# auduno/headtrackr

Hardware: NVIDIA H100
Metric: frames/sec @640x480 (detect+CAMShift) (higher is better)
Workload: dtype u8+f64

## Files before the change

headtrackr_b200/csrc/ht_api.cu:

```cuda
#include "../../include/headtrackr_b200.h"

#include <cuda.h>
#include <cuda_runtime.h>

#include <algorithm>
#include <cassert>
#include <cmath>
#include <cstdarg>
#include <cstddef>
#include <cstdio>
#include <cstdlib>
#include <cstring>
#include <map>
#include <memory>
#include <string>
#include <tuple>
#include <utility>
#include <vector>

#include "ht_common.cuh"
#include "ht_detect.cuh"
#include "ht_track.cuh"

using namespace ht;
// ... 507 lines not shown
  DevBuf d_tracker_state, d_tracker_params, d_tracker_events, d_tracker_wb;
  bool tracker_on = false;
  DevBuf d_debug, d_debug_tab;
  std::vector<DebugCanvas> h_debug;
  int debug_count = 0;
  int stroke_flags = 0, stroke_count = 0;
  DevBuf d_camera;
  std::vector<CameraCtl> h_camera;
  int camera_count = 0;
  DevBuf d_crop;
  std::vector<FaceCrop> h_crop;
  int crop_count = 0, crop_tiles = 0;
  DevBuf d_feed_table, d_feed_draw, d_feed_canvas;
  DevBuf d_ingest_recs;
  PinnedHost h_feed_table;
  Event feed_copied;
  DevBuf d_track_cost;
  DevBuf d_records, d_record_status;
  int track_heavy_div = 128;
  int track_heavy_cluster = 8;
  int track_mid_div = 32, track_mid_cluster = 4;
  Stream tier_stream[3];
  Event tier_done[3];
  int track_mask_frames = 4;
  int track_mask_min = 4;
  Event sched_ready;
  DevBuf d_sched;

  int fail(int code, const char *fmt, ...) {
    char buf[512];
    va_list ap; va_start(ap, fmt); vsnprintf(buf, sizeof(buf), fmt, ap); va_end(ap);
    err = buf;
    return code;
  }
};

#define CK(call)                                                                                   \
  do {                                                                                             \
    cudaError_t e_ = (call);                                                                       \
    if (e_ != cudaSuccess) return ctx->fail(HT_ERR_CUDA, "%s: %s", #call, cudaGetErrorString(e_)); \
  } while (0)

namespace {

bool is_device_ptr(const void *p) {
  if (!p) return false;
  cudaPointerAttributes a{};
  if (cudaPointerGetAttributes(&a, p) != cudaSuccess) { cudaGetLastError(); return false; }
// ... 96 lines not shown
  const bool on_device = is_device_ptr(slots);
  if (!on_device) {
    std::vector<uint8_t> seen((size_t)ctx->cfg.max_frames, 0);
    for (int i = 0; i < n; ++i) {
      if (slots[i] < 0 || slots[i] >= ctx->cfg.max_frames) return ctx->fail(HT_ERR_ARG, "slot %d out of range", slots[i]);
      if (seen[(size_t)slots[i]]++) return ctx->fail(HT_ERR_ARG, "slot %d appears twice in one batch", slots[i]);
    }
    CK(ctx->d_slots.reserve(sizeof(int32_t) * ctx->cfg.max_frames));
  }
  return stage_input(ctx, st, slots, on_device, sizeof(int32_t) * n, ctx->d_slots, d_slots);
}

int ensure_tracker_buffers(ht_ctx *ctx, cudaStream_t st) {
  const size_t mf = (size_t)ctx->cfg.max_frames;
  if (!ctx->model_hist.p) {
    CK(ctx->model_hist.reserve(mf * 4096 * sizeof(uint32_t)));
    CK(ctx->cur_hist.reserve(2 * mf * 4096 * sizeof(uint32_t)));
    CK(ctx->track_state.reserve(mf * sizeof(TrackState)));
    CK(cudaMemsetAsync(ctx->track_state.p, 0, mf * sizeof(TrackState), st));
    CK(ctx->d_rects.reserve(mf * 4 * sizeof(int32_t)));
    CK(ctx->d_found.reserve(mf * sizeof(int32_t)));
    CK(ctx->d_objs.reserve(mf * 6 * sizeof(int32_t)));
    CK(ctx->d_windows.reserve(mf * 4 * sizeof(int32_t)));
    CK(ctx->d_sched.reserve(2 * mf * sizeof(int32_t)));
    CK(ctx->d_track_cost.reserve(2 * mf * sizeof(int32_t)));
    CK(cudaMemsetAsync(ctx->d_track_cost.p, 0, 2 * mf * sizeof(int32_t), st));
    if (ctx->track_trace) {
      CK(ctx->d_trace.reserve(12 * mf * sizeof(unsigned long long)));
      CK(cudaMemsetAsync(ctx->d_trace.p, 0, 12 * mf * sizeof(unsigned long long), st));
    }
  }
  return HT_OK;
}

int launch_hist(ht_ctx *ctx, cudaStream_t st, const uint8_t *d_rgba, int n, int w, int h, uint32_t *hist, uint16_t *bins,
                const uint8_t *enable = nullptr) {
  const int n_px = w * h;
  int chunks = 1;
  if (n < 4 * ctx->sms) chunks = std::min(64, std::max(1, 8 * ctx->sms / n));
  if (chunks > 1) CK(cudaMemsetAsync(hist, 0, (size_t)n * 4096 * sizeof(uint32_t), st));
  ctx->prof_begin(HT_PROF_HIST, st);
  k_hist<<<dim3(chunks, n), 256, 0, st>>>(d_rgba, (size_t)n_px * 4, n_px, hist, bins, chunks, enable);
  ctx->prof_end(st);
  ++ctx->launches;
  CK(cudaGetLastError());
  return HT_OK;
}

using TrackKernel = void (*)(const uint16_t *, int, int, const int32_t *, const uint32_t *, const uint32_t *, TrackState *,
                             int, int32_t *, int32_t *, int32_t *, unsigned long long *, const int32_t *, int,
                             unsigned long long *, size_t, int, int, int32_t *, const uint8_t *);

template <int NT>
TrackKernel track_kernel(int c) {
  switch (c) {
    case 1: return k_track<1, NT>;
    case 2: return k_track<2, NT>;
    case 4: return k_track<4, NT>;
    case 16: return k_track<16, NT>;
    default: return k_track<8, NT>;
  }
}
TrackKernel track_kernel(int c, int nt) {
  return nt == 512 ? track_kernel<512>(c) : nt == 128 ? track_kernel<128>(c) : track_kernel<256>(c);
}

struct TrackArgs {
  const uint16_t *bins; int w, h; const int32_t *slots; const uint32_t *mh, *ch; TrackState *state; int n_calls;
  int32_t *objs, *win, *flag; unsigned long long *stats;
  unsigned long long *trace;
  size_t trace_stride;
  int memo;
  int force_serial;
  int32_t *cost;
  const uint8_t *enable;
};

cudaError_t launch_k_track(const TrackArgs &a, int c, int nt, cudaStream_t st, int n, const int32_t *order, int list_off) {
  if (c != 1 && c != 2 && c != 4 && c != 16) c = 8;
  if (nt != 128 && nt != 512) nt = 256;
  cudaLaunchConfig_t cfg{};
  cfg.gridDim = dim3((unsigned)n * c);
  cfg.blockDim = dim3(nt);
  cfg.dynamicSmemBytes = 0;
  cfg.stream = st;
  cudaLaunchAttribute attr[1];
  attr[0].id = cudaLaunchAttributeClusterDimension;
  attr[0].val.clusterDim.x = c; attr[0].val.clusterDim.y = 1; attr[0].val.clusterDim.z = 1;
  cfg.attrs = attr; cfg.numAttrs = 1;
  return cudaLaunchKernelEx(&cfg, track_kernel(c, nt), a.bins, a.w, a.h, a.slots, a.mh, a.ch, a.state, a.n_calls, a.objs,
                            a.win, a.flag, a.stats, order, list_off,
                            a.trace, a.trace_stride, a.memo, a.force_serial, a.cost, a.enable);
}

int launch_track(ht_ctx *ctx, cudaStream_t st, int n, int f0, const uint16_t *bins, int w, int h, const int32_t *d_slots,
                 const uint32_t *mh, const uint32_t *ch, TrackState *state, int n_calls, int32_t *d_objs, int32_t *d_win,
                 int32_t *flag, const uint8_t *enable = nullptr) {
  if (ctx->track_mask_min > 0 && n_calls >= ctx->track_mask_min) {
    const int chunks = std::max(1, std::min(64, 8 * ctx->sms / std::max(1, n)));
    const int min_px256 = (int)std::min<long long>(((long long)ctx->track_mask_frames * w * h) >> 8, 0x7fffffff);
    k_bins_mask<<<dim3((unsigned)chunks, (unsigned)n), 256, 0, st>>>(const_cast<uint16_t *>(bins), w * h, mh, d_slots, state, chunks, enable,
                                                                     ctx->track_mask_frames > 0 ? ctx->d_track_cost.as<int32_t>() : nullptr, min_px256);
    ++ctx->launches;
  }
  const TrackArgs args{bins, w, h, d_slots, mh, ch, state, n_calls, d_objs, d_win, flag,
                       ctx->d_flags.as<unsigned long long>() + 8,
                       ctx->track_trace ? ctx->d_trace.as<unsigned long long>() + 4 * (size_t)f0 : nullptr,
                       4 * (size_t)ctx->cfg.max_frames - 4 * (size_t)f0 + 8 * (size_t)f0,
                       ctx->track_memo ? 1 : 0, (ctx->force_ties & 4) ? 1 : 0, ctx->d_track_cost.as<int32_t>(), enable};
  cudaError_t e = cudaSuccess;
  int c = ctx->track_cluster;
  if (c <= 0) c = (n >= 256) ? 2 : (n >= 32 ? 4 : 8);
  if (n < 128) {
    e = launch_k_track(args, c, ctx->track_nt, st, n, nullptr, 0);
    ++ctx->launches;
  } else {
    int32_t *area = ctx->d_sched.as<int32_t>() + (size_t)f0;
    int32_t *order = ctx->d_sched.as<int32_t>() + (size_t)ctx->cfg.max_frames + f0;
    k_track_area<<<(n + 255) / 256, 256, 0, st>>>(state, d_slots, n, ctx->d_track_cost.as<int32_t>(), area);
    k_track_rank<<<(n + 255) / 256, 256, 0, st>>>(area, n, order);
    ctx->launches += 2;
    struct Tier { int count, cluster, threads, side; };
    Tier tiers[3];
    int n_tiers = 0, left = n;
    auto take = [&](int div, int cl, int side) {
      const int k = (div > 0) ? std::min(left, n / div) : 0;
      if (k > 0) { tiers[n_tiers++] = Tier{k, cl, 256, side}; left -= k; }
    };
    take(ctx->track_heavy_div, ctx->track_heavy_cluster, 0);
    take(ctx->track_mid_div, ctx->track_mid_cluster, 1);
    const bool rest_side = ctx->track_heavy_div > 0 || ctx->track_mid_div > 0;
    if (left > 0) tiers[n_tiers++] = Tier{left, c, ctx->track_nt, rest_side ? 2 : -1};
    if (n_tiers > 1) {
      int prio_least = 0, prio_greatest = 0;
      CK(cudaDeviceGetStreamPriorityRange(&prio_least, &prio_greatest));
      for (int t = 0; t < 3; ++t)
        if (!ctx->tier_stream[t]) {
          CK(cudaStreamCreateWithPriority(&ctx->tier_stream[t].h, cudaStreamNonBlocking, std::min(prio_least, prio_greatest + t)));
          CK(cudaEventCreateWithFlags(&ctx->tier_done[t].h, cudaEventDisableTiming));
        }
      if (!ctx->sched_ready) CK(cudaEventCreateWithFlags(&ctx->sched_ready.h, cudaEventDisableTiming));
      CK(cudaEventRecord(ctx->sched_ready, st));
    }
    int off = 0;
    for (int t = 0; t < n_tiers && e == cudaSuccess; ++t) {
      cudaStream_t ts = tiers[t].side >= 0 ? ctx->tier_stream[tiers[t].side] : st;
      if (tiers[t].side >= 0) CK(cudaStreamWaitEvent(ts, ctx->sched_ready, 0));
      e = launch_k_track(args, tiers[t].cluster, tiers[t].threads, ts, tiers[t].count, order, off);
      ++ctx->launches;
      if (tiers[t].side >= 0) CK(cudaEventRecord(ctx->tier_done[tiers[t].side], ts));
      off += tiers[t].count;
    }
    for (int t = 0; t < n_tiers; ++t)
      if (tiers[t].side >= 0) CK(cudaStreamWaitEvent(st, ctx->tier_done[tiers[t].side], 0));
  }
  if (e != cudaSuccess) return ctx->fail(HT_ERR_CUDA, "k_track launch: %s", cudaGetErrorString(e));
  return HT_OK;
}

int track_init_common(ht_ctx *ctx, cudaStream_t st, const int32_t *slots, int n, const uint8_t *d_rgba, int w, int h,
                      const int32_t *d_rects, int calc_angles, int32_t *out_found) {
  const int32_t *d_slots = nullptr;
  int rc = upload_slots(ctx, st, slots, n, &d_slots);
  if (rc != HT_OK) return rc;
  Outputs io(ctx);
  int32_t *d_found = io.out<int32_t>(out_found, ctx->d_found, sizeof(int32_t) * n);
  ctx->prof_begin(HT_PROF_TRACK_INIT, st);
  k_track_init<<<n, 256, 0, st>>>(d_rgba, (size_t)w * h * 4, w, h, d_slots, d_rects, calc_angles ? 1 : 0,
                                  ctx->model_hist.as<uint32_t>(), ctx->track_state.as<TrackState>(), d_found, nullptr);
  ctx->prof_end(st);
  ++ctx->launches;
  CK(cudaGetLastError());
  return io.finish(Outputs::SYNC_STREAM);
}

constexpr size_t CASC_SMEM = (size_t)TILE_WORDS * 4 + 3 * (size_t)MASK_WORDS * 32 * sizeof(uint32_t);
constexpr size_t GRAY_HIST_SMEM = 2 * 4096 * sizeof(uint32_t);

// ... 284 lines not shown
  if (const char *tm2 = getenv("HT_TRACK_MEMO")) c->track_memo = atoi(tm2) != 0;
  if (const char *tt = getenv("HT_TRACK_TRACE")) c->track_trace = atoi(tt) != 0;
  if (const char *tn = getenv("HT_TRACK_NT")) c->track_nt = (atoi(tn) == 128) ? 128 : (atoi(tn) == 512 ? 512 : 256);
  if (const char *th = getenv("HT_TRACK_HEAVY")) {
    c->track_heavy_div = std::max(0, atoi(th));
    if (const char *comma = strchr(th, ',')) {
      const int hc = atoi(comma + 1);
      if (hc == 1 || hc == 2 || hc == 4 || hc == 8 || hc == 16) c->track_heavy_cluster = hc;
    }
  }
  if (const char *tmid = getenv("HT_TRACK_MID")) {
    c->track_mid_div = std::max(0, atoi(tmid));
    if (const char *comma = strchr(tmid, ',')) {
      const int mc = atoi(comma + 1);
      if (mc == 2 || mc == 4 || mc == 8) c->track_mid_cluster = mc;
    }
  }
  if (const char *wv = getenv("HT_WAVE")) c->wave_frames = std::max(4, atoi(wv));
  if (const char *wm = getenv("HT_WAVE_MB")) c->wave_mb = std::max(1, atoi(wm));
  if (const char *tm = getenv("HT_TMA")) c->use_tma = atoi(tm) != 0;
  if (const char *ov = getenv("HT_OVERLAP")) { c->overlap_track = atoi(ov) != 0 ? 1 : 0; c->overlap_parts = atoi(ov); }
  if (const char *hc2 = getenv("HT_H2D_CHUNK")) c->h2d_chunk = std::max(1, atoi(hc2));
  if (const char *pl = getenv("HT_PIPELINE")) c->pipeline = atoi(pl) != 0 ? 1 : 0;
  if (const char *tk = getenv("HT_TRACK_MASK")) {
    c->track_mask_min = std::max(0, atoi(tk));
    if (const char *comma = strchr(tk, ',')) c->track_mask_frames = std::max(0, atoi(comma + 1));
  }
  if (cudaEventCreateWithFlags(&c->compute_done.h, cudaEventDisableTiming) != cudaSuccess) { g_create_error = "ht_create: event"; return HT_ERR_CUDA; }
  if (c->d_casc.reserve(c->hc.late.size() * sizeof(LateFeat)) != cudaSuccess ||
      cudaMemcpy(c->d_casc.p, c->hc.late.data(), c->hc.late.size() * sizeof(LateFeat), cudaMemcpyHostToDevice) != cudaSuccess ||
      c->d_late_chunk0.reserve(c->hc.late_chunk0.size() * sizeof(int32_t)) != cudaSuccess ||
      cudaMemcpy(c->d_late_chunk0.p, c->hc.late_chunk0.data(), c->hc.late_chunk0.size() * sizeof(int32_t), cudaMemcpyHostToDevice) != cudaSuccess) {
    g_create_error = "ht_create: cascade upload failed"; return HT_ERR_CUDA;
  }
  if (set_kernel_attributes(c.get()) != HT_OK) { g_create_error = "ht_create: " + c->err; return HT_ERR_CUDA; }
  const size_t mf = (size_t)cfg->max_frames;
  bool ok = c->raw_keys.reserve(mf * c->raw_cap * sizeof(uint32_t)) == cudaSuccess &&
            c->raw_conf.reserve(mf * c->raw_cap * sizeof(double)) == cudaSuccess &&
            c->raw_count.reserve(mf * sizeof(uint32_t)) == cudaSuccess &&
            c->sorted.reserve(mf * c->raw_cap * sizeof(Rect)) == cudaSuccess &&
            c->labels.reserve(mf * c->raw_cap * sizeof(int)) == cudaSuccess &&
            c->seq2.reserve(mf * c->raw_cap * sizeof(Rect)) == cudaSuccess &&
            c->d_out_rects.reserve(mf * c->K * sizeof(Rect)) == cudaSuccess &&
            c->d_out_counts.reserve(mf * sizeof(int32_t)) == cudaSuccess &&
            c->d_best.reserve(mf * sizeof(Rect)) == cudaSuccess &&
            c->d_flags.reserve(256) == cudaSuccess;
  if (!ok) { g_create_error = "ht_create: cudaMalloc failed"; return HT_ERR_CUDA; }
  cudaMemset(c->d_flags.p, 0, 256);
  cudaMemset(c->raw_count.p, 0, mf * sizeof(uint32_t));
  *out = c.release();
// ... 1756 lines not shown
  const HeadParams hp = make_head_params(params);
  HeadState s;
  head_new_state(s);
  for (int i = 0; i < n; ++i) {
    const double *c = cs + 5 * i;
    HeadEvent he;
    head_step(s, hp, c[0] != 0.0, c[1], c[2], c[3], c[4], c[0] != 0.0 && (c[3] == 0.0 || c[4] == 0.0), (double)camw, (double)camh, he);
    memcpy(out + i, &he, sizeof(he));
  }
  return 0;
}

extern "C" int ht_selftest_track_tolerance(const double *m, double n_px, double sw, double sh, int calc_angles, double *out) {
  const Mom mm = {m[0], m[1], m[2], m[3], m[4], m[5]};
  const TruncTol t = trunc_tolerance(mm, n_px, sw, sh, calc_angles != 0);
  out[0] = t.vx; out[1] = t.vy; out[2] = t.l1; out[3] = t.l2; out[4] = t.b;
  return 0;
}
extern "C" int ht_selftest_track_cap(int w, int h, double sw, double sh, double l1, double l2, double *out) {
  const TruncCap c = trunc_cap(w, h);
  out[0] = out[1] = shift_tolerance(c.eps, c.M, 0.5 * fmax(sw, sh));
  out[2] = c.root + 4.0 * TRUNC_U * l1; out[3] = c.root + 4.0 * TRUNC_U * l2; out[4] = c.b;
  return 0;
}

extern "C" int ht_selftest_tracker_size(void) { return (int)sizeof(TrackerState); }
extern "C" int ht_selftest_tracker(void *state, int op, const ht_tracker_params *params, double wb, const ht_rect *det,
                                   int count, const ht_trackobj *obj, double now_ms, int camw, int camh, ht_tracker_event *out,
                                   int32_t *seed) {
  TrackerState &s = *static_cast<TrackerState *>(state);
  if (op == 0) tracker_new_state(s);
  else if (op == 1) tracker_start(s);
  else if (op == 2) tracker_stop(s);
  else {
    const TrackerParams tp = make_tracker_params(params);
    int32_t zero_obj[6] = {0, 0, 0, 0, 0, 0};
    TrackerEvent e;
    bool sd;
    tracker_step(s, tp, wb, reinterpret_cast<const Rect *>(det), count, obj ? reinterpret_cast<const int32_t *>(obj) : zero_obj,
                 now_ms, (double)camw, (double)camh, e, seed + 1, sd);
    seed[0] = sd ? 1 : 0;
    memcpy(out, &e, sizeof(e));
  }
  return s.mode;
}

// ... 468 lines not shown
```

headtrackr_b200/csrc/ht_track.cuh:

```cuda
#pragma once
#include <cooperative_groups.h>

#include <cstring>
#include <limits>

#include "ht_common.cuh"

namespace ht {


__global__ void __launch_bounds__(256) k_hist(const uint8_t *__restrict__ rgba, size_t frame_bytes, int n_px,
                                              uint32_t *__restrict__ hist, uint16_t *__restrict__ bins, int chunks,
                                              const uint8_t *__restrict__ enable) {
  __shared__ uint32_t sh[4096];
  if (enable && !enable[blockIdx.y]) return;
  for (int i = threadIdx.x; i < 4096; i += 256) sh[i] = 0;
  __syncthreads();
  const uint32_t *px = reinterpret_cast<const uint32_t *>(rgba + (size_t)blockIdx.y * frame_bytes);
  uint16_t *bout = bins ? bins + (size_t)blockIdx.y * n_px : nullptr;
  const int n_pair = (n_px + 1) / 2;
  const int per = (n_pair + chunks - 1) / chunks;
  const int beg = blockIdx.x * per, end = min(n_pair, beg + per);
  const bool paired = ((reinterpret_cast<uintptr_t>(px) & 7u) == 0) && (!bout || (reinterpret_cast<uintptr_t>(bout) & 3u) == 0);
  for (int i = beg + threadIdx.x; i < end; i += 256) {
// ... 80 lines not shown
    if (cost) cost[2 * slot] = cost[2 * slot + 1] = 0;
  }
}

__global__ void k_pick_face(const Rect *__restrict__ det, int stride, const int32_t *__restrict__ counts, int cap, int n,
                            int32_t *__restrict__ rects) {
  const int k = blockIdx.x * blockDim.x + threadIdx.x;
  if (k >= n) return;
  const int c = min(counts[k], cap);
  int32_t r[4] = {0, 0, 0, 0};
  if (c > 0) {
    const Rect *d = det + (size_t)k * stride;
    int best = 0;
    for (int i = 1; i < c; ++i)
      if (d[i].confidence > d[best].confidence) best = i;
    if (d[best].confidence > -10.0) {
      r[0] = (int32_t)floor(d[best].x); r[1] = (int32_t)floor(d[best].y);
      r[2] = (int32_t)floor(d[best].width); r[3] = (int32_t)floor(d[best].height);
    }
  }
  rects[4 * k + 0] = r[0]; rects[4 * k + 1] = r[1]; rects[4 * k + 2] = r[2]; rects[4 * k + 3] = r[3];
}

constexpr uint32_t BIN_ZERO = 8u * 4096u;
constexpr uint32_t BIN_ZERO2 = BIN_ZERO | (BIN_ZERO << 16);
__global__ void __launch_bounds__(256) k_bins_mask(uint16_t *__restrict__ bins, int n_px, const uint32_t *__restrict__ model_hist,
                                                   const int32_t *__restrict__ slots, const TrackState *__restrict__ state,
                                                   int chunks, const uint8_t *__restrict__ enable,
                                                   const int32_t *__restrict__ cost, int min_px256) {
  __shared__ uint32_t bm[128];
  const int k = blockIdx.y;
  if (enable && !enable[k]) return;
  const int slot = slots ? slots[k] : k;
  if (!state[slot].initialised) return;
  if (cost && cost[2 * slot + 1] < min_px256) return;
  const uint32_t *mh = model_hist + (size_t)slot * 4096;
  if (threadIdx.x < 128) {
    uint32_t w = 0;
#pragma unroll 8
    for (int i = 0; i < 32; ++i) w |= (__ldg(mh + 32 * threadIdx.x + i) != 0u ? 1u : 0u) << i;
    bm[threadIdx.x] = w;
  }
  __syncthreads();
  uint16_t *pl = bins + (size_t)k * n_px;
  auto mask2 = [&](uint32_t v) {
    const uint32_t b0 = (v & 0xffffu) >> 3, b1 = v >> 19;
    uint32_t o = v;
    if (b0 < 4096u && !((bm[b0 >> 5] >> (b0 & 31u)) & 1u)) o = (o & 0xffff0000u) | BIN_ZERO;
    if (b1 < 4096u && !((bm[b1 >> 5] >> (b1 & 31u)) & 1u)) o = (o & 0x0000ffffu) | (BIN_ZERO << 16);
    return o;
  };
  const bool vec = ((reinterpret_cast<uintptr_t>(pl) & 15u) == 0);
  const int n_grp = vec ? n_px / 8 : 0;
  const int per = (n_grp + chunks - 1) / chunks;
  const int beg = blockIdx.x * per, end = min(n_grp, beg + per);
  for (int g = beg + threadIdx.x; g < end; g += 256) {
    uint4 v = *reinterpret_cast<const uint4 *>(pl + 8 * (size_t)g);
    const uint4 o = make_uint4(mask2(v.x), mask2(v.y), mask2(v.z), mask2(v.w));
    if (o.x != v.x || o.y != v.y || o.z != v.z || o.w != v.w) *reinterpret_cast<uint4 *>(pl + 8 * (size_t)g) = o;
  }
  if (blockIdx.x == 0)
    for (int p = 8 * n_grp + threadIdx.x; p < n_px; p += 256) {
      const uint32_t b = pl[p] >> 3;
      if (b < 4096u && !((bm[b >> 5] >> (b & 31u)) & 1u)) pl[p] = (uint16_t)BIN_ZERO;
    }
}


struct Mom {
  double m00, m10, m01, m11, m20, m02;
};

__device__ __forceinline__ int32_t js_to_int32(double v) {
  if (!isfinite(v)) return 0;
  return (int32_t)v;
}

__host__ __device__ __forceinline__ bool trunc_ambiguous(double v, double tol) {
  return isfinite(v) && fabs(v - rint(v)) < tol;
}

constexpr double TRUNC_U = 1.1102230246251565e-16;
__host__ __device__ __forceinline__ double sum_eps(double n_px) {
  const double nu = (n_px + 64.0) * TRUNC_U;
  return nu * (1.0 + 2.0 * nu) + TRUNC_U;
}
__host__ __device__ __forceinline__ double shift_tolerance(double eps, double xc, double half) {
  return 2.0 * (4.0 * eps * fabs(xc) + 2.0 * TRUNC_U * (fabs(xc) + half));
}
struct TruncTol { double vx, vy, l1, l2, b; };
// ... 38 lines not shown
  Mom m = {0, 0, 0, 0, 0, 0};
  for (int i = x; i < w; ++i) {
    const double vx = (double)(i - x);
    for (int j = y; j < h; ++j) {
      const double val = wsm[px[(size_t)j * W + i] >> 3];
      const double vy = (double)(j - y);
      m.m00 += val;
      m.m01 += vy * val;
      m.m10 += vx * val;
      m.m11 += vx * vy * val;
      m.m02 += vy * vy * val;
      m.m20 += vx * vx * val;
    }
  }
  return m;
}

__device__ __forceinline__ double warp_sum(double v) {
#pragma unroll
  for (int o = 16; o > 0; o >>= 1) v += __shfl_down_sync(0xffffffffu, v, o);
  return v;
}

constexpr int TRACK_CLUSTER_MAX = 16;

__global__ void k_track_area(const TrackState *__restrict__ state, const int32_t *__restrict__ slots, int n,
                             const int32_t *__restrict__ cost, int32_t *__restrict__ area) {
  const int i = blockIdx.x * blockDim.x + threadIdx.x;
  if (i >= n) return;
  const int slot = slots ? slots[i] : i;
  const TrackState *s = state + slot;
  long long a = 0;
  if (s->initialised) {
    const int passes = cost ? cost[2 * slot] : 0;
    if (passes > 0) a = 120ll * passes + cost[2 * slot + 1];
    else a = 120ll * 70 + 70ll * (((long long)max(s->sw, 0) * (long long)max(s->sh, 0)) >> 8);
  }
  area[i] = (int32_t)min(a, (long long)0x7fffffff);
}
__global__ void k_track_rank(const int32_t *__restrict__ area, int n, int32_t *__restrict__ order) {
  const int i = blockIdx.x * blockDim.x + threadIdx.x;
  if (i >= n) return;
  const int32_t a = area[i];
  int rank = 0;
  for (int j = 0; j < n; ++j) {
    const int32_t b = __ldg(area + j);
    rank += (b > a || (b == a && j < i)) ? 1 : 0;
  }
  order[rank] = i;
}

__device__ __forceinline__ double lds_f64(uint32_t saddr) {
  double v;
  asm volatile("ld.shared.f64 %0, [%1];" : "=d"(v) : "r"(saddr));
  return v;
}

__device__ __forceinline__ void row_partial(const uint16_t *__restrict__ row, const double *__restrict__ wsm, int lane,
                                            int wx, int xbeg, int xend, bool vec4, double &r0, double &r1, double &r2) {
  if (vec4) {
    for (int x4 = xbeg + 4 * lane; x4 < xend; x4 += 128) {
      const uint2 v = __ldg(reinterpret_cast<const uint2 *>(row + x4));
      const uint32_t b[4] = {(v.x & 0xffffu) >> 3, v.x >> 19, (v.y & 0xffffu) >> 3, v.y >> 19};
#pragma unroll
      for (int i = 0; i < 4; ++i) {
        const int x = x4 + i;
        const double val = (x >= wx && x < xend) ? wsm[b[i]] : 0.0;
        const double vx = (double)(x - wx);
        r0 += val;
        r1 += vx * val;
        r2 += (vx * vx) * val;
      }
    }
  } else {
    for (int x = wx + lane; x < xend; x += 32) {
      const double val = wsm[row[x] >> 3];
      const double vx = (double)(x - wx);
      r0 += val;
      r1 += vx * val;
      r2 += (vx * vx) * val;
    }
  }
}

template <int TRACK_CLUSTER, int NT>
__global__ void __launch_bounds__(NT, (NT >= 1024) ? 1 : (NT >= 512 ? 2 : (NT >= 256 ? 3 : 6)))
k_track(const uint16_t *__restrict__ bins, int W, int H, const int32_t *__restrict__ slots,
        const uint32_t *__restrict__ model_hist, const uint32_t *__restrict__ cur_hist, TrackState *__restrict__ state,
        int n_calls, int32_t *__restrict__ out_objs , int32_t *__restrict__ out_windows,
        int32_t *__restrict__ err_flag, unsigned long long *__restrict__ stats,
        const int32_t *__restrict__ order, int list_off,
        unsigned long long *__restrict__ trace, size_t trace_stride,
        int memo,
        int force_serial,
        int32_t *__restrict__ cost,
        const uint8_t *__restrict__ enable) {
  namespace cg = cooperative_groups;
  cg::cluster_group cluster = cg::this_cluster();
  __shared__ double wsm[4096 + 1];
  constexpr int NW = NT / 32;
  __shared__ double red[NW][6];
  __shared__ double cpart[2][TRACK_CLUSTER_MAX][6];
  __shared__ int win[4];
  __shared__ int ctrl;
  constexpr int MEMO_N = 8;
  struct MemoEnt { int w[4]; int exact; int valid; Mom m; };
  __shared__ MemoEnt memo_tab[MEMO_N];
  __shared__ int memo_next;
  __shared__ unsigned long long st_memo_sh;
  const int crank = (int)cluster.block_rank();
  int k = blockIdx.x / TRACK_CLUSTER;
  if (order) k = order[list_off + k];
  if (enable && !enable[k]) return;
  const int slot = slots ? slots[k] : k;
  const int tid = threadIdx.x, lane = tid & 31, warp = tid >> 5;
  const bool leader = (crank == 0 && tid == 0);
  const bool stepper = (tid == 0);
  struct Lead { TrackState s; unsigned long long st_pass, st_serial, st_px; int call, it, prevx, prevy;
                double shift_cap; };
  __shared__ Lead lead_sh;
  if (tid == 0) {
    lead_sh.s = state[slot];
    lead_sh.st_pass = lead_sh.st_serial = lead_sh.st_px = 0;
    lead_sh.call = 0; lead_sh.it = 0; lead_sh.prevx = lead_sh.s.sx; lead_sh.prevy = lead_sh.s.sy;
    memo_next = 0; st_memo_sh = 0;
    for (int i = 0; i < MEMO_N; ++i) memo_tab[i].valid = 0;
  }
  __syncthreads();
  TrackState &s = lead_sh.s;
  if (trace && leader) {
    unsigned long long t; unsigned smid;
    asm volatile("mov.u64 %0, %%globaltimer;" : "=l"(t));
    asm volatile("mov.u32 %0, %%smid;" : "=r"(smid));
    trace[4 * (size_t)k] = t; trace[4 * (size_t)k + 2] = smid;
  }
  if (!s.initialised) {
    if (leader) {
      atomicOr(err_flag, 1);
      int32_t *o = out_objs + 6 * (size_t)k;
      o[0] = o[1] = o[2] = o[3] = o[4] = o[5] = 0;
      if (out_windows) { int32_t *w4 = out_windows + 4 * (size_t)k; w4[0] = w4[1] = w4[2] = w4[3] = 0; }
    }
    return;
  }
  __shared__ double wmin[NW];
  __shared__ double nz_per_mass;
  __shared__ TruncCap cap;
  {
    const uint32_t *mh = model_hist + (size_t)slot * 4096, *ch = cur_hist + (size_t)k * 4096;
    double wm = INFINITY;
    for (int i = tid; i < 4096; i += NT) {
      const uint32_t c = ch[i], m = mh[i];
      double p = 0.0;
      if (c != 0 && m != 0) p = fmin((double)m / (double)c, 1.0);
      wsm[i] = p;
      if (p > 0.0) wm = fmin(wm, p);
    }
    if (tid == 0) wsm[4096] = 0.0;
#pragma unroll
    for (int o = 16; o > 0; o >>= 1) wm = fmin(wm, __shfl_xor_sync(0xffffffffu, wm, o));
    if (lane == 0) wmin[warp] = wm;
  }
  const uint16_t *px = bins + (size_t)k * W * H;
  const bool vec4 = (W & 3) == 0;
  int parity = 0;

  unsigned long long &st_pass = lead_sh.st_pass, &st_serial = lead_sh.st_serial, &st_px = lead_sh.st_px;
  double &shift_cap = lead_sh.shift_cap;
  int &call = lead_sh.call, &it = lead_sh.it, &prevx = lead_sh.prevx, &prevy = lead_sh.prevy;
  auto publish = [&](int done) {
    const int w0 = max(s.sx, 0), w1 = max(s.sy, 0);
    const int w2 = min(w0 + s.sw, W), w3 = min(w1 + s.sh, H);
    win[0] = w0; win[1] = w1; win[2] = w2; win[3] = w3;
    ctrl = done;
  };
  auto start_call = [&]() {
    if (call >= n_calls) return true;
// ... 9 lines not shown
  __syncthreads();
  if (stepper) {
    double wm = wmin[0];
    for (int i = 1; i < NW; ++i) wm = fmin(wm, wmin[i]);
    nz_per_mass = (1.0 + 1e-6) / wm;
  }

#ifndef HT_TRACK_PASSTRACE
#define HT_TRACK_PASSTRACE 0
#endif
#if HT_TRACK_PASSTRACE
  long long pt_acc[5] = {0, 0, 0, 0, 0};
  long long pt_t = 0;
#define HT_PT_MARK(i) do { if (trace && leader) { const long long now_ = clock64(); pt_acc[i] += now_ - pt_t; pt_t = now_; } } while (0)
#else
#define HT_PT_MARK(i) do { } while (0)
#endif
  constexpr int ROW_STRIDE = NW * TRACK_CLUSTER;
  while (!ctrl) {
    const int wx = win[0], wy = win[1], ww = win[2] - win[0], wh = win[3] - win[1];
#if HT_TRACK_PASSTRACE
    if (trace && leader) pt_t = clock64();
#endif
    double a00 = 0, a10 = 0, a01 = 0, a11 = 0, a20 = 0, a02 = 0;
    const int xbeg = wx & ~3, xend = wx + ww;
    const int mine = crank * NW + warp;
    const int yy0 = (mine - (wy % ROW_STRIDE) + ROW_STRIDE) % ROW_STRIDE;
    if (vec4) {
      const int n_x = (xend - xbeg + 127) >> 7;
      const int n_rg = (yy0 < wh) ? (wh - yy0 + 4 * ROW_STRIDE - 1) / (4 * ROW_STRIDE) : 0;
      const int total = n_rg * n_x;
      const uint16_t *col = px + (size_t)wy * W + xbeg + 4 * lane;
      const uint32_t wsm_base = (uint32_t)__cvta_generic_to_shared(wsm);
      constexpr uint32_t ZERO_W = 8u * 4096u;
      auto issue = [&](int rg, int xi, uint2 (&v)[4]) {
        const int x4 = xbeg + 4 * lane + 128 * xi;
#pragma unroll
        for (int j = 0; j < 4; ++j) {
          const int y = yy0 + (4 * rg + j) * ROW_STRIDE;
          v[j] = (y < wh && x4 < xend) ? __ldg(reinterpret_cast<const uint2 *>(col + (size_t)y * W + 128 * xi))
                                       : make_uint2(ZERO_W | (ZERO_W << 16), ZERO_W | (ZERO_W << 16));
        }
      };
      auto consume = [&](int rg, int xi, const uint2 (&v)[4]) {
        const int x4 = xbeg + 4 * lane + 128 * xi;
        double vx[4], vx2[4];
        bool in[4];
#pragma unroll
        for (int i = 0; i < 4; ++i) {
          const int x = x4 + i;
          in[i] = (x >= wx && x < xend);
          vx[i] = (double)(x - wx);
          vx2[i] = vx[i] * vx[i];
        }
#pragma unroll
        for (int j = 0; j < 4; ++j) {
          if (!__any_sync(0xffffffffu, v[j].x != BIN_ZERO2 || v[j].y != BIN_ZERO2)) continue;
          const int y = yy0 + (4 * rg + j) * ROW_STRIDE;
          const uint32_t b[4] = {v[j].x & 0xffffu, v[j].x >> 16, v[j].y & 0xffffu, v[j].y >> 16};
          double r0 = 0.0, r1 = 0.0, r2 = 0.0;
#pragma unroll
          for (int i = 0; i < 4; ++i) {
            const double val = lds_f64(wsm_base + (in[i] ? b[i] : ZERO_W));
            r0 += val;
            r1 = fma(vx[i], val, r1);
            r2 = fma(vx2[i], val, r2);
          }
          const double vy = (double)y;
          a00 += r0; a10 += r1; a20 += r2;
          a01 = fma(vy, r0, a01); a11 = fma(vy, r1, a11); a02 = fma(vy * vy, r0, a02);
        }
      };
      uint2 va[4], vb[4];
      int rg = 0, xi = 0;
      if (total > 0) issue(0, 0, va);
      for (int t = 0; t < total; t += 2) {
        int rg1 = rg, xi1 = xi + 1;
        if (xi1 == n_x) { xi1 = 0; ++rg1; }
        if (t + 1 < total) issue(rg1, xi1, vb);
        consume(rg, xi, va);
// ... 17 lines not shown
        for (int j = 0; j < 4; ++j) {
          const double vy = (double)(yy + j * ROW_STRIDE);
          a00 += r[j][0]; a10 += r[j][1]; a20 += r[j][2];
          a01 += vy * r[j][0]; a11 += vy * r[j][1]; a02 += (vy * vy) * r[j][0];
        }
      }
    }
    HT_PT_MARK(0);
    a00 = warp_sum(a00); a10 = warp_sum(a10); a01 = warp_sum(a01);
    a11 = warp_sum(a11); a20 = warp_sum(a20); a02 = warp_sum(a02);
    if (lane == 0) {
      red[warp][0] = a00; red[warp][1] = a10; red[warp][2] = a01;
      red[warp][3] = a11; red[warp][4] = a20; red[warp][5] = a02;
    }
    __syncthreads();
    HT_PT_MARK(1);
    if (tid < 6 * TRACK_CLUSTER) {
      const int q = tid % 6, r = tid / 6;
      double t = 0;
      for (int w8 = 0; w8 < NW; ++w8) t += red[w8][q];
      cluster.map_shared_rank(&cpart[0][0][0], r)[(parity * TRACK_CLUSTER_MAX + crank) * 6 + q] = t;
    }
    if (TRACK_CLUSTER > 1) cluster.sync(); else __syncthreads();
    HT_PT_MARK(2);
    if (stepper) {
      Mom m = {0, 0, 0, 0, 0, 0};
      for (int r = 0; r < TRACK_CLUSTER; ++r) {
        m.m00 += cpart[parity][r][0]; m.m10 += cpart[parity][r][1]; m.m01 += cpart[parity][r][2];
        m.m11 += cpart[parity][r][3]; m.m20 += cpart[parity][r][4]; m.m02 += cpart[parity][r][5];
      }
      bool exact = false;
      bool fresh = true;
      int cw0 = win[0], cw1 = win[1], cw2 = win[2], cw3 = win[3];
      ++st_pass;
      st_px += (unsigned long long)(max(ww, 0)) * (unsigned long long)(max(wh, 0));
      auto window_n = [&]() { return fmin((double)(cw2 - cw0) * (double)(cw3 - cw1), m.m00 * nz_per_mass); };
      for (;;) {
        double inv = 1.0 / m.m00;
        double vxf = m.m10 * inv - s.sw / 2.0, vyf = m.m01 * inv - s.sh / 2.0;
        bool amb_shift = force_serial;
        if (!exact && !amb_shift && (trunc_ambiguous(vxf, shift_cap) || trunc_ambiguous(vyf, shift_cap))) {
          const double eps = sum_eps(window_n());
          amb_shift = trunc_ambiguous(vxf, shift_tolerance(eps, m.m10 * inv, s.sw / 2.0)) ||
                      trunc_ambiguous(vyf, shift_tolerance(eps, m.m01 * inv, s.sh / 2.0));
        }
        if (!exact && amb_shift) {
// ... 1251 lines not shown
```

Baseline: 76590.

## Replace bin-masking pass with exact 128-bit row-prefix-sum moments for long CAMShift runs

Removes the k_bins_mask pre-pass. Frames whose tracking is expected to be expensive (many calls, large pixel cost, no angle calculation) now get per-row fixed-point 128-bit prefix sums of the weight, x-weight and x²-weight, built on a high-priority side stream. Each CAMShift pass then reads only two prefix entries per window row instead of every pixel, and the result stays exact because it is computed in integers and rounded once. This costs a large arena (up to 2 GiB), an extra build kernel that writes 48 bytes per pixel per stream, rank/area kernels that now also run for small batches, and slow emulated u128 arithmetic.

```diff
diff --git a/headtrackr_b200/csrc/ht_api.cu b/headtrackr_b200/csrc/ht_api.cu
--- a/headtrackr_b200/csrc/ht_api.cu
+++ b/headtrackr_b200/csrc/ht_api.cu
@@ -553,8 +553,11 @@
   int track_mid_div = 32, track_mid_cluster = 4;
   Stream tier_stream[3];
   Event tier_done[3];
-  int track_mask_frames = 4;
-  int track_mask_min = 4;
+  static constexpr int track_prefix_calls = 4, track_prefix_frames = 4;
+  static constexpr size_t track_prefix_bytes = size_t(2) << 30;
+  DevBuf d_prefix;
+  Stream prefix_stream;
+  Event prefix_done;
   Event sched_ready;
   DevBuf d_sched;
 
@@ -697,7 +700,7 @@
     CK(ctx->d_found.reserve(mf * sizeof(int32_t)));
     CK(ctx->d_objs.reserve(mf * 6 * sizeof(int32_t)));
     CK(ctx->d_windows.reserve(mf * 4 * sizeof(int32_t)));
-    CK(ctx->d_sched.reserve(2 * mf * sizeof(int32_t)));
+    CK(ctx->d_sched.reserve(3 * mf * sizeof(int32_t)));
     CK(ctx->d_track_cost.reserve(2 * mf * sizeof(int32_t)));
     CK(cudaMemsetAsync(ctx->d_track_cost.p, 0, 2 * mf * sizeof(int32_t), st));
     if (ctx->track_trace) {
@@ -724,7 +727,7 @@
 
 using TrackKernel = void (*)(const uint16_t *, int, int, const int32_t *, const uint32_t *, const uint32_t *, TrackState *,
                              int, int32_t *, int32_t *, int32_t *, unsigned long long *, const int32_t *, int,
-                             unsigned long long *, size_t, int, int, int32_t *, const uint8_t *);
+                             unsigned long long *, size_t, int, int, int32_t *, const uint8_t *, const u128 *);
 
 template <int NT>
 TrackKernel track_kernel(int c) {
@@ -750,6 +753,13 @@
   int32_t *cost;
   const uint8_t *enable;
 };
+
+cudaError_t launch_k_track_prefix(const TrackArgs &a, cudaStream_t st, int n, const int32_t *plist, const u128 *arena) {
+  k_track<1, 128, true><<<n, 128, 0, st>>>(a.bins, a.w, a.h, a.slots, a.mh, a.ch, a.state, a.n_calls, a.objs, a.win, a.flag,
+                                          a.stats, plist, 0, a.trace, a.trace_stride, a.memo, a.force_serial, a.cost,
+                                          a.enable, arena);
+  return cudaGetLastError();
+}
 
 cudaError_t launch_k_track(const TrackArgs &a, int c, int nt, cudaStream_t st, int n, const int32_t *order, int list_off) {
   if (c != 1 && c != 2 && c != 4 && c != 16) c = 8;
@@ -765,36 +775,59 @@
   cfg.attrs = attr; cfg.numAttrs = 1;
   return cudaLaunchKernelEx(&cfg, track_kernel(c, nt), a.bins, a.w, a.h, a.slots, a.mh, a.ch, a.state, a.n_calls, a.objs,
                             a.win, a.flag, a.stats, order, list_off,
-                            a.trace, a.trace_stride, a.memo, a.force_serial, a.cost, a.enable);
+                            a.trace, a.trace_stride, a.memo, a.force_serial, a.cost, a.enable, (const u128 *)nullptr);
 }
 
 int launch_track(ht_ctx *ctx, cudaStream_t st, int n, int f0, const uint16_t *bins, int w, int h, const int32_t *d_slots,
                  const uint32_t *mh, const uint32_t *ch, TrackState *state, int n_calls, int32_t *d_objs, int32_t *d_win,
                  int32_t *flag, const uint8_t *enable = nullptr) {
-  if (ctx->track_mask_min > 0 && n_calls >= ctx->track_mask_min) {
-    const int chunks = std::max(1, std::min(64, 8 * ctx->sms / std::max(1, n)));
-    const int min_px256 = (int)std::min<long long>(((long long)ctx->track_mask_frames * w * h) >> 8, 0x7fffffff);
-    k_bins_mask<<<dim3((unsigned)chunks, (unsigned)n), 256, 0, st>>>(const_cast<uint16_t *>(bins), w * h, mh, d_slots, state, chunks, enable,
-                                                                     ctx->track_mask_frames > 0 ? ctx->d_track_cost.as<int32_t>() : nullptr, min_px256);
-    ++ctx->launches;
-  }
   const TrackArgs args{bins, w, h, d_slots, mh, ch, state, n_calls, d_objs, d_win, flag,
                        ctx->d_flags.as<unsigned long long>() + 8,
                        ctx->track_trace ? ctx->d_trace.as<unsigned long long>() + 4 * (size_t)f0 : nullptr,
                        4 * (size_t)ctx->cfg.max_frames - 4 * (size_t)f0 + 8 * (size_t)f0,
                        ctx->track_memo ? 1 : 0, (ctx->force_ties & 4) ? 1 : 0, ctx->d_track_cost.as<int32_t>(), enable};
+  const bool force_prefix = (ctx->force_ties & 8) != 0;
+  const size_t prefix_stream_bytes = 3 * sizeof(u128) * (size_t)w * h;
+  int pcap = 0, min_px256 = -1;
+  if (prefix_fits(w, h) && (force_prefix || n_calls >= ctx->track_prefix_calls)) {
+    pcap = force_prefix ? n : (int)std::min<size_t>((size_t)n, ctx->track_prefix_bytes / prefix_stream_bytes);
+    min_px256 = force_prefix ? 0 : (int)std::min<long long>(((long long)ctx->track_prefix_frames * w * h) >> 8, 0x7fffffff);
+  }
+  int32_t *area = ctx->d_sched.as<int32_t>() + (size_t)f0;
+  int32_t *order = ctx->d_sched.as<int32_t>() + (size_t)ctx->cfg.max_frames + f0;
+  int32_t *plist = ctx->d_sched.as<int32_t>() + 2 * (size_t)ctx->cfg.max_frames + f0;
+  const bool ranked = n >= 128 || pcap > 0;
+  if (ranked) {
+    k_track_area<<<(n + 255) / 256, 256, 0, st>>>(state, d_slots, n, ctx->d_track_cost.as<int32_t>(), area, enable, min_px256);
+    k_track_rank<<<(n + 255) / 256, 256, 0, st>>>(area, n, order, pcap, plist);
+    ctx->launches += 2;
+  }
+  if (pcap > 0) {
+    CK(ctx->d_prefix.reserve(prefix_stream_bytes * pcap));
+    if (!ctx->prefix_stream) {
+      int prio_least = 0, prio_greatest = 0;
+      CK(cudaDeviceGetStreamPriorityRange(&prio_least, &prio_greatest));
+      CK(cudaStreamCreateWithPriority(&ctx->prefix_stream.h, cudaStreamNonBlocking, prio_greatest));
+      CK(cudaEventCreateWithFlags(&ctx->prefix_done.h, cudaEventDisableTiming));
+    }
+    if (!ctx->sched_ready) CK(cudaEventCreateWithFlags(&ctx->sched_ready.h, cudaEventDisableTiming));
+    CK(cudaEventRecord(ctx->sched_ready, st));
+    cudaStream_t ps = ctx->prefix_stream;
+    CK(cudaStreamWaitEvent(ps, ctx->sched_ready, 0));
+    k_track_prefix_build<<<dim3((unsigned)((h + 127) / 128), (unsigned)pcap), 128, 0, ps>>>(bins, w, h, d_slots, mh, ch, plist,
+                                                                                           ctx->d_prefix.as<u128>());
+    const cudaError_t e = launch_k_track_prefix(args, ps, pcap, plist, ctx->d_prefix.as<u128>());
+    if (e != cudaSuccess) return ctx->fail(HT_ERR_CUDA, "k_track prefix launch: %s", cudaGetErrorString(e));
+    ctx->launches += 2;
+    CK(cudaEventRecord(ctx->prefix_done, ps));
+  }
   cudaError_t e = cudaSuccess;
   int c = ctx->track_cluster;
   if (c <= 0) c = (n >= 256) ? 2 : (n >= 32 ? 4 : 8);
   if (n < 128) {
-    e = launch_k_track(args, c, ctx->track_nt, st, n, nullptr, 0);
+    e = launch_k_track(args, c, ctx->track_nt, st, n, ranked ? order : nullptr, 0);
     ++ctx->launches;
   } else {
-    int32_t *area = ctx->d_sched.as<int32_t>() + (size_t)f0;
-    int32_t *order = ctx->d_sched.as<int32_t>() + (size_t)ctx->cfg.max_frames + f0;
-    k_track_area<<<(n + 255) / 256, 256, 0, st>>>(state, d_slots, n, ctx->d_track_cost.as<int32_t>(), area);
-    k_track_rank<<<(n + 255) / 256, 256, 0, st>>>(area, n, order);
-    ctx->launches += 2;
     struct Tier { int count, cluster, threads, side; };
     Tier tiers[3];
     int n_tiers = 0, left = n;
@@ -815,7 +848,7 @@
           CK(cudaEventCreateWithFlags(&ctx->tier_done[t].h, cudaEventDisableTiming));
         }
       if (!ctx->sched_ready) CK(cudaEventCreateWithFlags(&ctx->sched_ready.h, cudaEventDisableTiming));
-      CK(cudaEventRecord(ctx->sched_ready, st));
+      if (pcap == 0) CK(cudaEventRecord(ctx->sched_ready, st));
     }
     int off = 0;
     for (int t = 0; t < n_tiers && e == cudaSuccess; ++t) {
@@ -829,6 +862,7 @@
     for (int t = 0; t < n_tiers; ++t)
       if (tiers[t].side >= 0) CK(cudaStreamWaitEvent(st, ctx->tier_done[tiers[t].side], 0));
   }
+  if (pcap > 0) CK(cudaStreamWaitEvent(st, ctx->prefix_done, 0));
   if (e != cudaSuccess) return ctx->fail(HT_ERR_CUDA, "k_track launch: %s", cudaGetErrorString(e));
   return HT_OK;
 }
@@ -1159,10 +1193,6 @@
   if (const char *ov = getenv("HT_OVERLAP")) { c->overlap_track = atoi(ov) != 0 ? 1 : 0; c->overlap_parts = atoi(ov); }
   if (const char *hc2 = getenv("HT_H2D_CHUNK")) c->h2d_chunk = std::max(1, atoi(hc2));
   if (const char *pl = getenv("HT_PIPELINE")) c->pipeline = atoi(pl) != 0 ? 1 : 0;
-  if (const char *tk = getenv("HT_TRACK_MASK")) {
-    c->track_mask_min = std::max(0, atoi(tk));
-    if (const char *comma = strchr(tk, ',')) c->track_mask_frames = std::max(0, atoi(comma + 1));
-  }
   if (cudaEventCreateWithFlags(&c->compute_done.h, cudaEventDisableTiming) != cudaSuccess) { g_create_error = "ht_create: event"; return HT_ERR_CUDA; }
   if (c->d_casc.reserve(c->hc.late.size() * sizeof(LateFeat)) != cudaSuccess ||
       cudaMemcpy(c->d_casc.p, c->hc.late.data(), c->hc.late.size() * sizeof(LateFeat), cudaMemcpyHostToDevice) != cudaSuccess ||
@@ -2965,6 +2995,36 @@
   out[0] = out[1] = shift_tolerance(c.eps, c.M, 0.5 * fmax(sw, sh));
   out[2] = c.root + 4.0 * TRUNC_U * l1; out[3] = c.root + 4.0 * TRUNC_U * l2; out[4] = c.b;
   return 0;
+}
+
+extern "C" int ht_selftest_track_prefix(const uint16_t *bins, int w, int h, const uint32_t *mh, const uint32_t *ch, int x0,
+                                        int y0, int x1, int y1, int32_t *info, double *m) {
+  info[0] = prefix_scale(w, h);
+  info[1] = prefix_fits(w, h) ? 1 : 0;
+  if (!info[1]) return -1;
+  const int s = info[0];
+  std::vector<u128> row(3 * (size_t)w);
+  u128 a[6] = {0, 0, 0, 0, 0, 0};
+  for (int y = y0; y < y1; ++y) {
+    u128 c0 = 0, c1 = 0, c2 = 0;
+    for (int x = 0; x < w; ++x) {
+      const int b = bins[(size_t)y * w + x] >> 3;
+      const u128 q = prefix_fixed(track_weight(mh[b], ch[b]), s);
+      c0 += q; c1 += q * (u128)x; c2 += q * (u128)x * (u128)x;
+      row[3 * (size_t)x] = c0; row[3 * (size_t)x + 1] = c1; row[3 * (size_t)x + 2] = c2;
+    }
+    if (x1 > x0) {
+      const u128 hi[3] = {row[3 * (size_t)(x1 - 1)], row[3 * (size_t)(x1 - 1) + 1], row[3 * (size_t)(x1 - 1) + 2]};
+      u128 lo[3] = {0, 0, 0};
+      if (x0 > 0) for (int q = 0; q < 3; ++q) lo[q] = row[3 * (size_t)(x0 - 1) + q];
+      prefix_row(hi, lo, x0, y - y0, a);
+    }
+  }
+  for (int q = 0; q < 6; ++q) m[q] = prefix_to_double(a[q], s);
+  return 0;
+}
+extern "C" double ht_selftest_prefix_round(uint64_t hi, uint64_t lo, int s) {
+  return prefix_to_double(((u128)hi << 64) | lo, s);
 }
 
 extern "C" int ht_selftest_tracker_size(void) { return (int)sizeof(TrackerState); }
diff --git a/headtrackr_b200/csrc/ht_track.cuh b/headtrackr_b200/csrc/ht_track.cuh
--- a/headtrackr_b200/csrc/ht_track.cuh
+++ b/headtrackr_b200/csrc/ht_track.cuh
@@ -126,50 +126,6 @@
   rects[4 * k + 0] = r[0]; rects[4 * k + 1] = r[1]; rects[4 * k + 2] = r[2]; rects[4 * k + 3] = r[3];
 }
 
-constexpr uint32_t BIN_ZERO = 8u * 4096u;
-constexpr uint32_t BIN_ZERO2 = BIN_ZERO | (BIN_ZERO << 16);
-__global__ void __launch_bounds__(256) k_bins_mask(uint16_t *__restrict__ bins, int n_px, const uint32_t *__restrict__ model_hist,
-                                                   const int32_t *__restrict__ slots, const TrackState *__restrict__ state,
-                                                   int chunks, const uint8_t *__restrict__ enable,
-                                                   const int32_t *__restrict__ cost, int min_px256) {
-  __shared__ uint32_t bm[128];
-  const int k = blockIdx.y;
-  if (enable && !enable[k]) return;
-  const int slot = slots ? slots[k] : k;
-  if (!state[slot].initialised) return;
-  if (cost && cost[2 * slot + 1] < min_px256) return;
-  const uint32_t *mh = model_hist + (size_t)slot * 4096;
-  if (threadIdx.x < 128) {
-    uint32_t w = 0;
-#pragma unroll 8
-    for (int i = 0; i < 32; ++i) w |= (__ldg(mh + 32 * threadIdx.x + i) != 0u ? 1u : 0u) << i;
-    bm[threadIdx.x] = w;
-  }
-  __syncthreads();
-  uint16_t *pl = bins + (size_t)k * n_px;
-  auto mask2 = [&](uint32_t v) {
-    const uint32_t b0 = (v & 0xffffu) >> 3, b1 = v >> 19;
-    uint32_t o = v;
-    if (b0 < 4096u && !((bm[b0 >> 5] >> (b0 & 31u)) & 1u)) o = (o & 0xffff0000u) | BIN_ZERO;
-    if (b1 < 4096u && !((bm[b1 >> 5] >> (b1 & 31u)) & 1u)) o = (o & 0x0000ffffu) | (BIN_ZERO << 16);
-    return o;
-  };
-  const bool vec = ((reinterpret_cast<uintptr_t>(pl) & 15u) == 0);
-  const int n_grp = vec ? n_px / 8 : 0;
-  const int per = (n_grp + chunks - 1) / chunks;
-  const int beg = blockIdx.x * per, end = min(n_grp, beg + per);
-  for (int g = beg + threadIdx.x; g < end; g += 256) {
-    uint4 v = *reinterpret_cast<const uint4 *>(pl + 8 * (size_t)g);
-    const uint4 o = make_uint4(mask2(v.x), mask2(v.y), mask2(v.z), mask2(v.w));
-    if (o.x != v.x || o.y != v.y || o.z != v.z || o.w != v.w) *reinterpret_cast<uint4 *>(pl + 8 * (size_t)g) = o;
-  }
-  if (blockIdx.x == 0)
-    for (int p = 8 * n_grp + threadIdx.x; p < n_px; p += 256) {
-      const uint32_t b = pl[p] >> 3;
-      if (b < 4096u && !((bm[b >> 5] >> (b & 31u)) & 1u)) pl[p] = (uint16_t)BIN_ZERO;
-    }
-}
-
 
 struct Mom {
   double m00, m10, m01, m11, m20, m02;
@@ -254,32 +210,123 @@
   return v;
 }
 
+__host__ __device__ __forceinline__ double track_weight(uint32_t m, uint32_t c) {
+  return (c != 0 && m != 0) ? fmin((double)m / (double)c, 1.0) : 0.0;
+}
+
+using u128 = unsigned __int128;
+
+__host__ __device__ inline int prefix_scale(int W, int H) {
+  const long long n = (long long)W * (long long)H;
+  int L = 0;
+  while ((1ll << L) < n) ++L;
+  return L + 52;
+}
+__host__ __device__ inline bool prefix_fits(int W, int H) {
+  if (W <= 0 || H <= 0) return false;
+  const u128 M = (u128)(W > H ? W : H);
+  const u128 bound = (u128)W * (u128)H * M * M;
+  const int s = prefix_scale(W, H);
+  return s < 127 && (bound >> (127 - s)) == 0;
+}
+__host__ __device__ __forceinline__ u128 prefix_fixed(double w, int s) {
+  if (!(w > 0.0)) return 0;
+#ifdef __CUDA_ARCH__
+  const uint64_t bits = (uint64_t)__double_as_longlong(w);
+#else
+  uint64_t bits;
+  memcpy(&bits, &w, 8);
+#endif
+  const uint64_t mant = (bits & ((1ull << 52) - 1)) | (1ull << 52);
+  return (u128)mant << ((int)(bits >> 52) - 1075 + s);
+}
+__host__ __device__ __forceinline__ double prefix_to_double(u128 v, int s) {
+  const uint64_t hi = (uint64_t)(v >> 64), lo = (uint64_t)v;
+  if (hi == 0) return ldexp((double)lo, -s);
+#ifdef __CUDA_ARCH__
+  const int sh = 64 - __clzll((long long)hi);
+#else
+  const int sh = 64 - __builtin_clzll(hi);
+#endif
+  const uint64_t top = (uint64_t)(v >> sh) | ((lo << (64 - sh)) != 0 ? 1u : 0u);
+  return ldexp((double)top, sh - s);
+}
+__host__ __device__ __forceinline__ void prefix_row(const u128 (&hi)[3], const u128 (&lo)[3], int x0, int vy, u128 (&a)[6]) {
+  const u128 r0 = hi[0] - lo[0], r1 = hi[1] - lo[1], r2 = hi[2] - lo[2];
+  const u128 X = (u128)x0;
+  const u128 q1 = r1 - X * r0, q2 = r2 - 2 * X * r1 + X * X * r0, Y = (u128)vy;
+  a[0] += r0; a[1] += q1; a[2] += Y * r0; a[3] += Y * q1; a[4] += q2; a[5] += Y * Y * r0;
+}
+
+__global__ void __launch_bounds__(128) k_track_prefix_build(const uint16_t *__restrict__ bins, int W, int H,
+                                                             const int32_t *__restrict__ slots,
+                                                             const uint32_t *__restrict__ model_hist,
+                                                             const uint32_t *__restrict__ cur_hist,
+                                                             const int32_t *__restrict__ plist, u128 *__restrict__ arena) {
+  __shared__ double wsm[4096];
+  const int k = plist[blockIdx.y];
+  if (k < 0) return;
+  const int slot = slots ? slots[k] : k;
+  const uint32_t *mh = model_hist + (size_t)slot * 4096, *ch = cur_hist + (size_t)k * 4096;
+  for (int i = threadIdx.x; i < 4096; i += 128) wsm[i] = track_weight(mh[i], ch[i]);
+  __syncthreads();
+  const int y = blockIdx.x * 128 + threadIdx.x;
+  if (y >= H) return;
+  const int s = prefix_scale(W, H);
+  const size_t plane = (size_t)W * H;
+  const uint16_t *row = bins + (size_t)k * plane + (size_t)y * W;
+  u128 *p0 = arena + (size_t)blockIdx.y * 3 * plane + y, *p1 = p0 + plane, *p2 = p1 + plane;
+  u128 c0 = 0, c1 = 0, c2 = 0;
+  for (int x = 0; x < W; ++x) {
+    const u128 q = prefix_fixed(wsm[row[x] >> 3], s);
+    c0 += q;
+    c1 += q * (u128)x;
+    c2 += q * (u128)((uint64_t)x * (uint64_t)x);
+    const size_t i = (size_t)x * H;
+    p0[i] = c0; p1[i] = c1; p2[i] = c2;
+  }
+}
+
 constexpr int TRACK_CLUSTER_MAX = 16;
 
 __global__ void k_track_area(const TrackState *__restrict__ state, const int32_t *__restrict__ slots, int n,
-                             const int32_t *__restrict__ cost, int32_t *__restrict__ area) {
+                             const int32_t *__restrict__ cost, int32_t *__restrict__ area, const uint8_t *__restrict__ enable,
+                             int min_px256) {
   const int i = blockIdx.x * blockDim.x + threadIdx.x;
   if (i >= n) return;
   const int slot = slots ? slots[i] : i;
   const TrackState *s = state + slot;
   long long a = 0;
+  bool prefix = false;
   if (s->initialised) {
+    prefix = min_px256 >= 0 && (!enable || enable[i]) &&
+             (min_px256 == 0 || (!s->calc_angles && cost && cost[2 * slot + 1] >= min_px256));
     const int passes = cost ? cost[2 * slot] : 0;
     if (passes > 0) a = 120ll * passes + cost[2 * slot + 1];
     else a = 120ll * 70 + 70ll * (((long long)max(s->sw, 0) * (long long)max(s->sh, 0)) >> 8);
   }
-  area[i] = (int32_t)min(a, (long long)0x7fffffff);
-}
-__global__ void k_track_rank(const int32_t *__restrict__ area, int n, int32_t *__restrict__ order) {
+  a = min(a, (long long)0x7fffffff);
+  area[i] = (int32_t)(prefix ? a - 0x80000000ll : a);
+}
+__global__ void k_track_rank(const int32_t *__restrict__ area, int n, int32_t *__restrict__ order, int cap,
+                             int32_t *__restrict__ plist) {
   const int i = blockIdx.x * blockDim.x + threadIdx.x;
   if (i >= n) return;
   const int32_t a = area[i];
-  int rank = 0;
+  int rank = 0, n_pre = 0;
   for (int j = 0; j < n; ++j) {
     const int32_t b = __ldg(area + j);
     rank += (b > a || (b == a && j < i)) ? 1 : 0;
-  }
-  order[rank] = i;
+    n_pre += b < 0 ? 1 : 0;
+  }
+  const int pos = rank - (n - n_pre);
+  if (pos >= 0 && pos < cap) {
+    plist[pos] = i;
+    order[rank] = -1;
+  } else {
+    order[rank] = i;
+  }
+  if (i < cap && i >= n_pre) plist[i] = -1;
 }
 
 __device__ __forceinline__ double lds_f64(uint32_t saddr) {
@@ -315,8 +362,8 @@
   }
 }
 
-template <int TRACK_CLUSTER, int NT>
-__global__ void __launch_bounds__(NT, (NT >= 1024) ? 1 : (NT >= 512 ? 2 : (NT >= 256 ? 3 : 6)))
+template <int TRACK_CLUSTER, int NT, bool PREFIX = false>
+__global__ void __launch_bounds__(NT, PREFIX ? 4 : ((NT >= 1024) ? 1 : (NT >= 512 ? 2 : (NT >= 256 ? 3 : 6))))
 k_track(const uint16_t *__restrict__ bins, int W, int H, const int32_t *__restrict__ slots,
         const uint32_t *__restrict__ model_hist, const uint32_t *__restrict__ cur_hist, TrackState *__restrict__ state,
         int n_calls, int32_t *__restrict__ out_objs , int32_t *__restrict__ out_windows,
@@ -326,12 +373,15 @@
         int memo,
         int force_serial,
         int32_t *__restrict__ cost,
-        const uint8_t *__restrict__ enable) {
+        const uint8_t *__restrict__ enable,
+        const u128 *__restrict__ prefix) {
+  static_assert(!PREFIX || TRACK_CLUSTER == 1, "the prefix path runs one CTA per stream");
   namespace cg = cooperative_groups;
   cg::cluster_group cluster = cg::this_cluster();
   __shared__ double wsm[4096 + 1];
   constexpr int NW = NT / 32;
   __shared__ double red[NW][6];
+  __shared__ u128 red128[PREFIX ? NW : 1][6];
   __shared__ double cpart[2][TRACK_CLUSTER_MAX][6];
   __shared__ int win[4];
   __shared__ int ctrl;
@@ -343,6 +393,7 @@
   const int crank = (int)cluster.block_rank();
   int k = blockIdx.x / TRACK_CLUSTER;
   if (order) k = order[list_off + k];
+  if (k < 0) return;
   if (enable && !enable[k]) return;
   const int slot = slots ? slots[k] : k;
   const int tid = threadIdx.x, lane = tid & 31, warp = tid >> 5;
@@ -382,9 +433,7 @@
     const uint32_t *mh = model_hist + (size_t)slot * 4096, *ch = cur_hist + (size_t)k * 4096;
     double wm = INFINITY;
     for (int i = tid; i < 4096; i += NT) {
-      const uint32_t c = ch[i], m = mh[i];
-      double p = 0.0;
-      if (c != 0 && m != 0) p = fmin((double)m / (double)c, 1.0);
+      const double p = track_weight(mh[i], ch[i]);
       wsm[i] = p;
       if (p > 0.0) wm = fmin(wm, p);
     }
@@ -440,6 +489,44 @@
 #if HT_TRACK_PASSTRACE
     if (trace && leader) pt_t = clock64();
 #endif
+    if constexpr (PREFIX) {
+      u128 a[6] = {0, 0, 0, 0, 0, 0};
+      const size_t plane = (size_t)W * H;
+      const u128 *pre = prefix + (size_t)blockIdx.x * 3 * plane;
+      const u128 *ehi = pre + (size_t)(wx + ww - 1) * H + wy, *elo = pre + (size_t)max(wx - 1, 0) * H + wy;
+      auto load = [&](int yy, u128 (&hi)[3], u128 (&lo)[3]) {
+#pragma unroll
+        for (int q = 0; q < 3; ++q) {
+          hi[q] = ehi[q * plane + yy];
+          lo[q] = wx > 0 ? elo[q * plane + yy] : (u128)0;
+        }
+      };
+      if (ww > 0)
+        for (int yy = tid; yy < wh; yy += 2 * NT) {
+          u128 hi[3], lo[3], hi2[3] = {0, 0, 0}, lo2[3] = {0, 0, 0};
+          load(yy, hi, lo);
+          if (yy + NT < wh) load(yy + NT, hi2, lo2);
+          prefix_row(hi, lo, wx, yy, a);
+          prefix_row(hi2, lo2, wx, yy + NT, a);
+        }
+#pragma unroll
+      for (int q = 0; q < 6; ++q) {
+#pragma unroll
+        for (int o = 16; o > 0; o >>= 1) {
+          const uint64_t lo = __shfl_xor_sync(0xffffffffu, (uint64_t)a[q], o);
+          const uint64_t hi = __shfl_xor_sync(0xffffffffu, (uint64_t)(a[q] >> 64), o);
+          a[q] += ((u128)hi << 64) | lo;
+        }
+        if (lane == 0) red128[warp][q] = a[q];
+      }
+      __syncthreads();
+      if (tid < 6) {
+        u128 t = 0;
+        for (int w8 = 0; w8 < NW; ++w8) t += red128[w8][tid];
+        cpart[parity][0][tid] = prefix_to_double(t, prefix_scale(W, H));
+      }
+      __syncthreads();
+    } else {
     double a00 = 0, a10 = 0, a01 = 0, a11 = 0, a20 = 0, a02 = 0;
     const int xbeg = wx & ~3, xend = wx + ww;
     const int mine = crank * NW + warp;
@@ -451,13 +538,14 @@
       const uint16_t *col = px + (size_t)wy * W + xbeg + 4 * lane;
       const uint32_t wsm_base = (uint32_t)__cvta_generic_to_shared(wsm);
       constexpr uint32_t ZERO_W = 8u * 4096u;
+      constexpr uint32_t ZERO_W2 = ZERO_W | (ZERO_W << 16);
       auto issue = [&](int rg, int xi, uint2 (&v)[4]) {
         const int x4 = xbeg + 4 * lane + 128 * xi;
 #pragma unroll
         for (int j = 0; j < 4; ++j) {
           const int y = yy0 + (4 * rg + j) * ROW_STRIDE;
           v[j] = (y < wh && x4 < xend) ? __ldg(reinterpret_cast<const uint2 *>(col + (size_t)y * W + 128 * xi))
-                                       : make_uint2(ZERO_W | (ZERO_W << 16), ZERO_W | (ZERO_W << 16));
+                                       : make_uint2(ZERO_W2, ZERO_W2);
         }
       };
       auto consume = [&](int rg, int xi, const uint2 (&v)[4]) {
@@ -473,7 +561,7 @@
         }
 #pragma unroll
         for (int j = 0; j < 4; ++j) {
-          if (!__any_sync(0xffffffffu, v[j].x != BIN_ZERO2 || v[j].y != BIN_ZERO2)) continue;
+          if (!__any_sync(0xffffffffu, v[j].x != ZERO_W2 || v[j].y != ZERO_W2)) continue;
           const int y = yy0 + (4 * rg + j) * ROW_STRIDE;
           const uint32_t b[4] = {v[j].x & 0xffffu, v[j].x >> 16, v[j].y & 0xffffu, v[j].y >> 16};
           double r0 = 0.0, r1 = 0.0, r2 = 0.0;
@@ -537,6 +625,7 @@
       cluster.map_shared_rank(&cpart[0][0][0], r)[(parity * TRACK_CLUSTER_MAX + crank) * 6 + q] = t;
     }
     if (TRACK_CLUSTER > 1) cluster.sync(); else __syncthreads();
+    }
     HT_PT_MARK(2);
     if (stepper) {
       Mom m = {0, 0, 0, 0, 0, 0};
```

Result: faster. 80230 (median of 6 runs) (+4.8%).
